# nekopanda/Amatsukaze

Hardware: AMD Instinct MI355X
Metric: frames/sec 1440x1080i logo+CM+KFM pass (higher is better)
Workload: dtype f32; 1 GPU; configs[1]: 10000x 1440x1080i 8-bit in HBM: AMTAnalyzeLogo, LogoFrame scan x3, CM/KFM metrics, CalcFade, AMTEraseLogo; analysis_mode=linear, library_default_mode=exact, calc_fade=device, erase=into a resident writable copy (MakeWritable's frame), frames_per_gpu=10000, logo=256x128@(1120,64), parallelism=single GPU

## Files before the change

### amatsukaze_amd/csrc/eval_engine.hip

```cpp
#include "build_knobs.h"
#include "engine.hpp"

#include <algorithm>
#include <cmath>
#include <cstdio>
#include <cstdlib>
#include <cstring>

int AmtGpuContext::prof_id(const char* name)
{
    for (size_t i = 0; i < prof_names.size(); ++i) if (prof_names[i] == name) return (int)i;
    prof_names.push_back(name);
    prof_ms.push_back(0.0);
    prof_calls.push_back(0);
    return (int)prof_names.size() - 1;
}
hipEvent_t AmtGpuContext::prof_event()
{
    if (!prof_pool.empty()) { hipEvent_t e = prof_pool.back(); prof_pool.pop_back(); return e; }
    hipEvent_t e;
    AMT_HIP(hipEventCreate(&e));
    return e;
}
int AmtGpuContext::prof_begin(const char* name)
// ... 89 lines not shown
                if ((slot_y(e) + 2 - ytop + 1) * lpb > kPlaneCapMax) break;
                minx = mnx; maxx = mxx;
                B.x0 = x0; B.bw = x1 - x0; B.lp = lpb;
                ++e;
            }
            if (e == s) throw std::runtime_error("logo too wide for the evaluation kernel");
            B.nslots = e - s;
            B.y0 = ytop;
            B.nrows = slot_y(e - 1) + 2 - ytop + 1;
            B.m0 = slot_m0(s);
            B.npix = slot_m0(e - 1) + (int)(slots[e - 1] >> 28) - B.m0;
            plane_cap_ = std::max(plane_cap_, B.nrows * B.lp);
            bands_.push_back(B);
            s = e;
        }

        std::vector<float2> scales((size_t)kNumBins * cpad, float2{0.0f, 0.0f});
        for (int m = 0; m < T.count; ++m)
            for (int c = 0; c < kNumBins; ++c)
                scales[(size_t)c * cpad + m] = float2{T.scales[((size_t)m * 32 + c) * 2], T.scales[((size_t)m * 32 + c) * 2 + 1]};
        const int spad = std::max(64, (ns + 63) / 64 * 64);
        std::vector<float2> kslot((size_t)25 * spad, float2{0.0f, 0.0f});
        std::vector<uint2> slot2(spad, uint2{0u, 0u});
        for (int bi = band0; bi < (int)bands_.size(); ++bi) {
            const EvalBand& B = bands_[bi];
            for (int sidx = B.s0; sidx < B.s0 + B.nslots; ++sidx) {
                const int m0 = slot_m0(sidx);
                const int n = (int)(slots[sidx] >> 28);
                const int x = (int)(T.pos[m0] & 0xFFFF), y = (int)(T.pos[m0] >> 16);
                slot2[sidx] = uint2{slots[sidx], (uint32_t)((y - 2 - B.y0) * B.lp + (x - 2 - B.x0))};
                const float* k0 = &T.kernels[(size_t)m0 * 25];
                const float* k1 = n > 1 ? &T.kernels[(size_t)(m0 + 1) * 25] : nullptr;
                for (int c = 0; c < 5; ++c)
                    for (int r = 0; r < 5; ++r) {
                        const float a0 = c < 4 ? k0[r * 5 + c + 1] : k0[r * 5];
                        const float a1 = k1 ? (c < 4 ? k1[r * 5 + c] : k1[r * 5 + 4]) : 0.0f;
                        kslot[(size_t)(c * 5 + r) * spad + sidx] = float2{a0, a1};
                    }
            }
        }
        d_a_[i].upload(S.planes.A(0), (size_t)w * h, ctx_->stream);
        d_b_[i].upload(S.planes.B(0), (size_t)w * h, ctx_->stream);
        d_scales_[i].upload(scales, ctx_->stream);
        d_kslot_[i].upload(kslot, ctx_->stream);
        d_slot2_[i].upload(slot2, ctx_->stream);

        EvalLogoDev& D = hl[i];
        D.a = d_a_[i].get(); D.b = d_b_[i].get(); D.scales = d_scales_[i].get();
        D.kslot = d_kslot_[i].get(); D.slot2 = d_slot2_[i].get(); D.nslots_pad = spad;
        D.band0 = band0; D.nbands = (int)bands_.size() - band0;
        D.w = w; D.h = h; D.count = T.count; D.count_pad = cpad;
        D.imgx = S.imgx; D.imgy = S.imgy; D.row0 = S.row0; D.row_step = S.row_step; D.deint = S.deint;
        D.blackScore = T.blackScore;
        D.out_off = S.out_off;
        D.lp = lp;
    }
#ifdef AMT_EXPERIMENT
    if (std::getenv("AMTGPU_VERBOSE")) {
        for (int i = 0; i < nl; ++i)
            fprintf(stderr, "[amtgpu] eval logo %d: %dx%d count=%d bands=%d lp=%d\n", i, hl[i].w, hl[i].h, hl[i].count, hl[i].nbands, hl[i].lp);
        for (const EvalBand& B : bands_)
            fprintf(stderr, "[amtgpu]   band logo=%d slots=%d npix=%d y0=%d nrows=%d x0=%d bw=%d lp=%d\n", B.logo, B.nslots, B.npix, B.y0, B.nrows, B.x0, B.bw, B.lp);
    }
#endif
    d_logos_.upload(hl, ctx_->stream);
    d_bands_.upload(bands_, ctx_->stream);
    d_fades_.upload(fades_, ctx_->stream);
}

double EvalEngine::mask_pixel_evals_per_frame() const
{
    double s = 0;
    for (const auto& sp : specs_) s += (double)sp.tables.count * fades_.size();
    return s;
}

void EvalEngine::run(const void* dY, int64_t frame_stride_bytes, int pitch, int bits, int nframes, float* dout,
                     const int* dframe_map)
{
    if (nframes <= 0 || specs_.empty()) return;
    ctx_->bind();
    const int es = bits <= 8 ? 1 : 2;
    if (frame_stride_bytes % es) throw std::runtime_error("frame stride not a multiple of the sample size");
    const int nl = (int)specs_.size();
    int G = exact_group_frames(nframes);
    const int nf_all = (int)fades_.size();
    if (pair_eligible() && pair_addressable(pitch * es)) {
        const size_t dot = prof_name_.find('.');
        const int sp = ctx_->prof_begin(("logo_eval_pair_kernel" + (dot == std::string::npos ? std::string() : prof_name_.substr(dot))).c_str());
        const int Gp = group_frames_ > 0 ? group_frames_ : (int)std::max(1LL, std::min((long long)kTileMaxFrames, (long long)nframes * nl / 2048));
        AMT_HIP(launch_logo_eval_pair(ctx_->stream, bits, d_logos_.get(), d_tls_.get(), nl, dY, dframe_map,
                                      frame_stride_bytes / es, pitch, nframes, Gp, dout, out_frame_stride_, take_abs_ ? 1 : 0));
        ctx_->prof_end(sp);
        return;
    }
    for (int f0 = 0; f0 < nf_all; f0 += kEvalMaxFades) {
        const int nf = std::min(kEvalMaxFades, nf_all - f0);
        G = std::max(1, std::min(G, kEvalThreads / nf));
        const int sp = ctx_->prof_begin(prof_name_.c_str());
        AMT_HIP(launch_logo_eval_fused(ctx_->stream, bits, d_logos_.get(), nl, d_bands_.get(), d_fades_.get(), nf, f0, dY, dframe_map,
                                       frame_stride_bytes / es, pitch, nframes, G, dout, out_frame_stride_, take_abs_ ? 1 : 0,
                                       plane_cap_));
        ctx_->prof_end(sp);
    }
}

int EvalEngine::exact_group_frames(int nframes) const
{
    const int nl = (int)specs_.size();
    return group_frames_ > 0 ? group_frames_ : (int)std::max(1LL, std::min(8LL, (long long)nframes * nl / 2048));
}

bool EvalEngine::pair_eligible()
{
    if (pair_state_ >= 0) return pair_state_ == 1;
    pair_state_ = 0;
#ifdef AMT_EXPERIMENT
    if (std::getenv("AMTGPU_NO_PAIR")) return false;
#endif
    if (fades_.size() != 2 || fades_[0] != 0.0f || fades_[1] != 1.0f || specs_.empty()) return false;
    for (const EvalLogoSpec& S : specs_) {
        const int w = S.planes.w, h = S.planes.h;
        if (w < 6 || (w & 1) || h < 5 || S.tables.count <= 0 || S.tables.count >= (1 << 20)) return false;
        if (!S.deint) return false;
        const float* a = S.planes.A(0);
        const float* b = S.planes.B(0);
        for (int p = 0; p < w * h; ++p)
            if (!(std::fabs(a[p]) + std::fabs(b[p]) < 8192.0f)) return false;
    }
    ensure_tiles();
    pair_state_ = 1;
    return true;
}

bool EvalEngine::pair_addressable(int pitch_bytes) const
{
    for (const EvalLogoSpec& S : specs_) {
        const long long last = (long long)(S.imgy + S.row0 + (long long)S.planes.h * S.row_step + 1) * pitch_bytes + (long long)(S.imgx + S.planes.w) * 2;
        if (last >= (1LL << 31) || pitch_bytes <= 0) return false;
    }
    return true;
}

void EvalEngine::ensure_tiles()
{
    if (tiles_ready_) return;
    ctx_->bind();
    const int nl = (int)specs_.size();
    std::vector<TileLogoDev> hl(nl);
    d_tkp_.resize(nl); d_tsc_.resize(nl); d_tpq_.resize(nl); d_tinfo_.resize(nl); d_tpos_.resize(nl); d_tlin_.resize(nl); d_tiles_.resize(nl); d_tbands_.resize(nl); d_tlist_.resize(nl);
    for (int i = 0; i < nl; ++i) {
        const EvalLogoSpec& S = specs_[i];
        const MaskTables& T = S.tables;
        const TilePlan P = build_tile_plan(T.pos, T.count, S.planes.w, S.planes.h);
        const size_t ns = (size_t)P.nslots();
        std::vector<float2> kp(13 * ns, float2{0.0f, 0.0f}), sc((size_t)kNumBins * ns, float2{0.0f, 0.0f}), pq(ns, float2{0.0f, 0.0f});
        std::vector<uint32_t> spos(ns, 0u);
        for (size_t s = 0; s < ns; ++s) {
            const int m = P.slot_pixel[s];
            if (m < 0) continue;
            fit_response(&T.resp[(size_t)m * 32], pq[s].x, pq[s].y);
            spos[s] = T.pos[m];
            const float* k = &T.kernels[(size_t)m * 25];
            float ksum = 0.0f;
            for (int t = 0; t < 25; ++t) ksum += k[t];
            for (int j = 0; j < 13; ++j) kp[(size_t)j * ns + s] = float2{k[2 * j], 2 * j + 1 < 25 ? k[2 * j + 1] : ksum};
            for (int c = 0; c < kNumBins; ++c)
                sc[(size_t)c * ns + s] = float2{T.scales[((size_t)m * 32 + c) * 2], T.scales[((size_t)m * 32 + c) * 2 + 1]};
        }
        d_tkp_[i].upload(kp, ctx_->stream);
        d_tsc_[i].upload(sc, ctx_->stream);
        d_tpq_[i].upload(pq, ctx_->stream);
        d_tpos_[i].upload(spos, ctx_->stream);
        const size_t npx = (size_t)S.planes.w * S.planes.h;
        const size_t o_pq = kp.size() * sizeof(float2), o_si = o_pq + pq.size() * sizeof(float2), o_a = o_si + P.sinfo.size() * sizeof(uint32_t),
                     o_b = o_a + npx * sizeof(float), total = o_b + npx * sizeof(float);
        if (total >= ((size_t)1 << 31)) throw std::runtime_error("logo too large");
        std::vector<char> blob(total);
        std::memcpy(blob.data(), kp.data(), o_pq);
        std::memcpy(blob.data() + o_pq, pq.data(), o_si - o_pq);
        std::memcpy(blob.data() + o_si, P.sinfo.data(), o_a - o_si);
        std::memcpy(blob.data() + o_a, S.planes.A(0), npx * sizeof(float));
        std::memcpy(blob.data() + o_b, S.planes.B(0), npx * sizeof(float));
        d_tlin_[i].upload(blob, ctx_->stream);
        d_tinfo_[i].upload(P.sinfo, ctx_->stream);
        d_tiles_[i].upload(P.tiles, ctx_->stream);
        d_tbands_[i].upload(P.bands, ctx_->stream);
        std::vector<int> tlist;
        for (size_t t = 0; t < P.tiles.size(); ++t) if (P.tiles[t].npix > 0) tlist.push_back((int)t);
        d_tlist_[i].upload(tlist, ctx_->stream);
        hl[i] = TileLogoDev{d_tkp_[i].get(), d_tsc_[i].get(), d_tpq_[i].get(), d_tinfo_[i].get(), d_tpos_[i].get(), d_tiles_[i].get(), d_tbands_[i].get(), d_tlist_[i].get(),
                            (int)P.bands.size(), (int)ns, (int)tlist.size(), T.floorResp};
        hl[i].lin = d_tlin_[i].get();
        hl[i].lin_pq = (unsigned)o_pq; hl[i].lin_sinfo = (unsigned)o_si; hl[i].lin_a = (unsigned)o_a; hl[i].lin_b = (unsigned)o_b;
    }
    d_tls_.upload(hl, ctx_->stream);
    tiles_ready_ = true;
}

void EvalEngine::ensure_linear()
{
    if (linear_ready_) return;
    const int nl = (int)specs_.size();
    lin_err_corr_.assign(nl, 0.0); lin_err_sum_.assign(nl, 0.0); lin_err_formula_.assign(nl, 0.0);
    lin_formula_ok_ = true;
    double vunit = 1.0;
    for (int i = 0; i < nl; ++i) {
        const EvalLogoSpec& S = specs_[i];
        const MaskTables& T = S.tables;
        const int w = S.planes.w, h = S.planes.h;
        const float* a = S.planes.A(0);
        const float* b = S.planes.B(0);
        for (int p = 0; p < w * h; ++p) {
            const double ab = (double)std::fabs(a[p]) + std::fabs(b[p]);
            if (!(ab < 1e30)) throw std::runtime_error("logo coefficients are not finite: the linear mode has no error bound for them");
            vunit = std::max(vunit, ab);
        }
        const double L = T.floorResp;
        if (!(L > 1e-20 && L < 1e30) || T.resp.size() != (size_t)T.count * 32) lin_formula_ok_ = false;
        double ecorr = 0, tsum = 0, eformula = 0;
        for (int m = 0; m < T.count; ++m) {
            double sk = 0;
            for (int t = 0; t < 25; ++t) sk += std::fabs(T.kernels[(size_t)m * 25 + t]);
            double smax = 0, s2max = 0, devmax = 0;
            float Pf = 0.0f, Qf = 0.0f;
            if (lin_formula_ok_) fit_response(&T.resp[(size_t)m * 32], Pf, Qf);
            if (!(std::fabs(Pf) < 1e30f && std::fabs(Qf) < 1e30f)) lin_formula_ok_ = false;
            for (int c = 0; c < kNumBins; ++c) {
                const double sc = std::fabs(T.scales[((size_t)m * 32 + c) * 2]), s2 = std::fabs(T.scales[((size_t)m * 32 + c) * 2 + 1]);
                smax = std::max(smax, sc * s2);
                s2max = std::max(s2max, s2);
                if (!lin_formula_ok_) continue;
                const double rk = formula_response(Pf, Qf, c), dk = std::max(rk, L);
                const auto tref = [&](double x) { return std::min(1.0, x * sc) * s2; };
                const auto tker = [&](double x) { return std::min(x, rk) / dk; };
                double dev = std::fabs((sc > 0 ? s2 : 0.0) - rk / dk);
                dev = std::max(dev, std::fabs(tref(rk) - tker(rk)));
                if (sc > 0) dev = std::max(dev, std::fabs(tref(1.0 / sc) - tker(1.0 / sc)));
                devmax = std::max(devmax, dev);
                smax = std::max(smax, 1.0 / dk);
                s2max = std::max(s2max, rk / dk);
            }
            eformula += devmax;
            ecorr += smax * sk * (58.0 + 24.0);
            tsum += s2max;
        }
        const double black = std::max(1e-30, (double)std::fabs(T.blackScore));
        lin_err_corr_[i] = ecorr / black;
        lin_err_sum_[i] = ((double)T.count + 52.0) * tsum / black + 8.0;
        lin_err_formula_[i] = eformula / black;
    }
    bool unit_fades = true;
    for (float f : fades_) unit_fades = unit_fades && f >= 0.0f && f <= 1.0f;
    vmax_unit_ = (float)(vunit * (unit_fades ? 1.0 : 2.0));
    linear_ready_ = true;
}

bool EvalEngine::tiles_usable(int pitch_bytes) const
{
    for (const EvalLogoSpec& S : specs_) {
        const int w = S.planes.w, h = S.planes.h;
        if (w < 6 || (w & 1) || h < 5 || S.tables.count <= 0 || S.tables.count >= 900000) return false;
    }
    return pair_addressable(pitch_bytes);
}

float EvalEngine::linear_error_bound(int logo, int bits) const
{
    const_cast<EvalEngine*>(this)->ensure_linear();
    const double u = 1.0 / 16777216.0, maxv = (double)((1 << bits) - 1);
    return (float)(1.25 * (u * (lin_err_corr_[logo] * vmax_unit_ * maxv + lin_err_sum_[logo]) + lin_err_formula_[logo]));
}

void EvalEngine::run_linear(const void* dY, int64_t frame_stride_bytes, int pitch, int bits, int nframes, float* dout, const int* dframe_map,
                            uint8_t* dforce)
{
    if (nframes <= 0 || specs_.empty()) return;
    const int es = bits <= 8 ? 1 : 2;
    if ((int)fades_.size() != 11 || fades_.front() != 0.0f || fades_.back() != 1.0f || !tiles_usable(pitch * es)) { run(dY, frame_stride_bytes, pitch, bits, nframes, dout, dframe_map); return; }
    ensure_linear();
    if (!lin_formula_ok_) { run(dY, frame_stride_bytes, pitch, bits, nframes, dout, dframe_map); return; }
    ensure_tiles();
    ctx_->bind();
    if (frame_stride_bytes % es) throw std::runtime_error("frame stride not a multiple of the sample size");
    const int nl = (int)specs_.size();
    const double vwin = (double)vmax_unit_ * (double)((1 << bits) - 1);
    const float bin_eps = (float)(22.0 / 16777216.0 * vwin * 1.0001);
    int qlog2 = 24;
    while (qlog2 > 4 && std::ldexp(vwin, qlog2) >= 1073741824.0) --qlog2;
    if (!(std::ldexp(vwin, qlog2) < 1073741824.0)) { run(dY, frame_stride_bytes, pitch, bits, nframes, dout, dframe_map); return; }
    const int qcap = std::max(16, std::min(640, lin_queue_));
    const int g_fit = (int)((160 * 1024 / 4 - 16 * 1024 - 4 * 8 * qcap - 16) / (4 * 768));
    if (g_fit < 1) { run(dY, frame_stride_bytes, pitch, bits, nframes, dout, dframe_map); return; }
    const int gmax = std::min(g_fit, bits > 8 ? kLinMaxFrames16 : kLinMaxFrames);
    const long long wgs_min = bits > 8 ? AMT_LIN_WGS_MIN16 : 2048;
    const int G = std::min(gmax, group_frames_ > 0 ? group_frames_ : (int)std::max(1LL, std::min(16LL, (long long)nframes * nl / wgs_min)));
    const size_t dot = prof_name_.find('.');
    const int sp = ctx_->prof_begin(("logo_eval_linear_kernel" + (dot == std::string::npos ? std::string() : prof_name_.substr(dot))).c_str());
    AMT_HIP(launch_logo_eval_linear(ctx_->stream, bits, d_logos_.get(), d_tls_.get(), nl, d_fades_.get(), 11, 0, dY, dframe_map,
                                    frame_stride_bytes / es, pitch, nframes, G, dout, out_frame_stride_, take_abs_ ? 1 : 0, bin_eps, qlog2,
                                    qcap, dforce));
    ctx_->prof_end(sp);
}

#ifndef AMT_LISTED_FADE_CHUNK
#define AMT_LISTED_FADE_CHUNK 1
#endif
// ... 23 lines not shown
```

### amatsukaze_amd/csrc/eval_pair_kernels.hip

```cpp
#include "build_knobs.h"
#include <hip/hip_runtime.h>
#include <cstdint>
#include <algorithm>

#include "engine.hpp"
#include "eval_tiles.hpp"
#include "exact_math.h"
#include "eval_tile_stage.h"
#include "eval_ordered_sum.h"

namespace amt {

using namespace lin;
using namespace tile;

constexpr int kPairThreads = (kTileWaves + 1) * 64;
constexpr int kPairRowPitch = kTileBandPix + kEvalScorePad;

__device__ __forceinline__ f2 window_corr_exact(const f2 (&Kp)[13], const f2 (&W)[25], f2 M)
{
    f2 p[5];
#pragma unroll
    for (int i = 0; i < 5; ++i) {
        f2 t[5];
#pragma unroll
        for (int r = 0; r < 5; ++r) {
            const int e = r * 5 + i;
            const f2 kk = (e & 1) ? bc_hi(Kp[e >> 1]) : bc_lo(Kp[e >> 1]);
            t[r] = kk * (W[e] - M);
        }
        p[i] = ((t[0] + t[1]) + (t[2] + t[3])) + t[4];
    }
    return ((p[0] + p[4]) + p[2]) + (p[1] + p[3]);
}

__device__ __forceinline__ unsigned score_bin_bounded(float mean) { return (unsigned)((int)__builtin_amdgcn_fmed3f(mean, 0.0f, 255.0f) >> 3); }

struct PairLaunch {
    const EvalLogoDev* logos;
    const TileLogoDev* tls;
    const void* Y;
    const int* frame_map;
    long long frame_stride;
    int pitch;
    float maxv;
    int nframes, G, ngroups, nlogos;
    float* out;
    int out_frame_stride, take_abs;
};

#ifdef AMT_PAIR_OCC
#define AMT_PAIR_OCC_ATTR __attribute__((amdgpu_waves_per_eu(AMT_PAIR_OCC, AMT_PAIR_OCC)))
#else
#define AMT_PAIR_OCC_ATTR
#endif
template <typename pix_t>
__global__ __launch_bounds__(kPairThreads) AMT_PAIR_OCC_ATTR
void logo_eval_pair_kernel(const PairLaunch A)
{
    extern __shared__ float lds[];
    f2* const planes = reinterpret_cast<f2*>(lds);
    float* const rows = lds + kTileWaves * kTileCap * 2;

#ifdef AMT_PAIR_TIMING
    long long tacc[8] = {0, 0, 0, 0, 0, 0, 0, 0};
    long long tprev = clock64();
#define AMT_PTICK(k) do { const long long t_ = clock64(); tacc[k] += t_ - tprev; tprev = t_; } while (0)
#define AMT_PDUMP() do { if (lane == 0 && logo == 0 && grp == A.ngroups / 2) { \
        long long* tb = reinterpret_cast<long long*>(A.out + (long long)A.nframes * A.out_frame_stride);    \
        for (int k = 0; k < 8; ++k) tb[wave * 8 + k] = tacc[k]; \
        tb[16 * 8 + wave] = __builtin_amdgcn_s_getreg((4 << 0) | (0 << 6) | (31 << 11));    } } while (0)
#else
#define AMT_PTICK(k) do { } while (0)
#define AMT_PDUMP() do { } while (0)
#endif
    const int G = A.G;
    const WgMap wm = wg_map_shared_rows((int)blockIdx.x, A.nlogos, A.ngroups);
    if (wm.grp >= A.ngroups) return;
    const int logo = wm.logo, grp = wm.grp;
    const int F0 = grp * G;
    const int gcount = min(G, A.nframes - F0);
    const int tid = threadIdx.x, lane = tid & 63;
    const int wave = __builtin_amdgcn_readfirstlane(tid >> 6);
    const EvalLogoDev* const Lp = A.logos + logo;
    const TileLogoDev* const Xp = A.tls + logo;
    const int nbands = Xp->nbands;
    constexpr int ES = (int)sizeof(pix_t);

    if (wave == kTileWaves) {
        __builtin_amdgcn_s_setprio(3);
        float acc = 0.0f;
        typedef const __attribute__((address_space(4))) TileBandDesc* const_band_ptr;
        const const_band_ptr bd = (const_band_ptr)Xp->bands;
        for (int b = 0; b < nbands; ++b) {
            asm volatile("s_waitcnt lgkmcnt(0)\n\ts_barrier" ::: "memory");
            AMT_PTICK(5);
            const int npix = bd[b].npix;
#ifndef AMT_PAIR_NO_SUM
            if (lane < 2 * gcount) acc = ordered_row_sum(rows + ((b & 1) * 2 * G + lane) * kPairRowPitch, npix, acc);
#endif
#ifdef AMT_PAIR_TIMING
            asm volatile("" : "+v"(acc));
#endif
            AMT_PTICK(0);
        }
        if (lane < 2 * gcount) {
            float r = acc / Lp->blackScore;
            if (A.take_abs) r = fabsf(r);
            A.out[(long long)(F0 + (lane >> 1)) * A.out_frame_stride + Lp->out_off + (lane & 1)] = r;
        }
        AMT_PDUMP();
        return;
    }

    const gptr_t gSc = (gptr_t)Xp->sc;
    const unsigned nslots8 = (unsigned)Xp->nslots * 8u;
    const const_tile_ptr tiles = (const_tile_ptr)(Xp->tiles + wave);
    f2* const myplane = planes + wave * kTileCap;
    const unsigned plane_base = lds_address(myplane);
    TileStager<pix_t> st;
    st.init(Lp, A.pitch, A.maxv, myplane);
    TilePixel px;

    TileDesc T;
    fetch_tile(T, tiles);
    st.setup_units(T, lane);
    st.request(frame_rsrc<pix_t>(A.Y, A.frame_map, A.frame_stride, F0));
    asm volatile("" ::: "memory");
    px.load(Xp, (unsigned)wave * 64u + (unsigned)lane, T, plane_base);

    f2 pR = {0.0f, 0.0f}, psc0 = pR, psc1 = pR;
    int prow = 0;
    bool pact = false;
    auto flush_terms = [&]() {
        if (pact) {
            float* const pdst = rows + prow * kPairRowPitch + px.ridx;
            pdst[0] = score_term(pR.x, psc0.x, psc0.y);
            pdst[kPairRowPitch] = score_term(pR.y, psc1.x, psc1.y);
        }
    };

    int b = 0, g = 0;
    const int niter = nbands * gcount;
    for (int it = 0; it < niter; ++it) {
        const bool band_end = g + 1 == gcount;
        AMT_PTICK(6);
#ifdef AMT_PAIR_TIMING
        asm volatile("s_waitcnt vmcnt(2)" ::: "memory");
        AMT_PTICK(7);
#endif
#ifndef AMT_PAIR_NO_CONVERT
        st.convert();
#endif
        AMT_PTICK(0);
        if (band_end && b + 1 < nbands) {
            fetch_tile(T, tiles + (b + 1) * kTileWaves);
            st.setup_units(T, lane);
        }
#if defined(AMT_PAIR_RAW_SAMEFRAME)
        st.request(frame_rsrc<pix_t>(A.Y, A.frame_map, A.frame_stride, 0));
#elif !defined(AMT_PAIR_NO_RAW)
        st.request(frame_rsrc<pix_t>(A.Y, A.frame_map, A.frame_stride, F0 + (band_end ? 0 : g + 1)));
#endif
        AMT_PTICK(1);
#pragma unroll
        for (int j = 0; j < 13; ++j) asm volatile("" : "+v"(px.Kp[j]));
        f2 W[25];
        unsigned wrow[5];
        px.rows(wrow);
#ifdef AMT_PAIR_NO_EVAL
        const f2 M = px.Kp[1] + f2{100.0f, 120.0f}, R = px.Kp[0];
        (void)W;
#else
        const f2 M = window_load_means(wrow, W);
        const f2 R = window_corr_exact(px.Kp, W, M);
#endif
#ifdef AMT_PAIR_TIMING
        { f2 Rt = R; asm volatile("" : "+v"(Rt)); }
#endif
        AMT_PTICK(2);
#ifndef AMT_PAIR_NO_FLUSH
        flush_terms();
#endif
#ifdef AMT_PAIR_NO_GATHER
        psc0 = f2{1e-3f, 1.0f} + M; psc1 = f2{1e-3f, 1.0f} - M;
#else
        psc0 = gld<f2>(gSc, __umul24(score_bin_bounded(M.x), nslots8) + px.slot8);
        psc1 = gld<f2>(gSc, __umul24(score_bin_bounded(M.y), nslots8) + px.slot8);
#endif
        pR = R; pact = px.act;
        AMT_PTICK(3);
        prow = (b & 1) * 2 * G + g * 2;
        if (band_end) {
            flush_terms();
            pact = false;
            ++b; g = 0;
            if (b < nbands) px.load(Xp, (unsigned)(b * kTileWaves + wave) * 64u + (unsigned)lane, T, plane_base);
            AMT_PTICK(4);
            asm volatile("s_waitcnt lgkmcnt(0)\n\ts_barrier" ::: "memory");
            AMT_PTICK(5);
        } else {
            ++g;
        }
    }
    AMT_PDUMP();
}

hipError_t launch_logo_eval_pair(hipStream_t st, int bits, const EvalLogoDev* dlogos, const TileLogoDev* dtls, int nlogos,
                                 const void* dY, const int* dframe_map, long long frame_stride_elems, int pitch,
                                 int nframes, int G, float* dout, int out_frame_stride, int take_abs)
{
    if (nframes <= 0 || nlogos <= 0) return hipSuccess;
    PairLaunch A;
    A.logos = dlogos; A.tls = dtls; A.Y = dY; A.frame_map = dframe_map; A.frame_stride = frame_stride_elems; A.pitch = pitch;
    A.maxv = (float)((1 << bits) - 1);
    A.nframes = nframes; A.G = G; A.ngroups = (nframes + G - 1) / G; A.nlogos = nlogos;
    A.out = dout; A.out_frame_stride = out_frame_stride; A.take_abs = take_abs;
    const size_t lds = ((size_t)kTileWaves * kTileCap * 2 + (size_t)2 * 2 * G * kPairRowPitch) * sizeof(float);
    if (G < 1 || 2 * G > 64 || lds > 160 * 1024) return hipErrorInvalidValue;
    dim3 grid((unsigned)wg_grid_shared_rows(A.ngroups, nlogos));
    if (bits <= 8) hipLaunchKernelGGL(logo_eval_pair_kernel<uint8_t>, grid, dim3(kPairThreads), lds, st, A);
    else hipLaunchKernelGGL(logo_eval_pair_kernel<uint16_t>, grid, dim3(kPairThreads), lds, st, A);
    return hipGetLastError();
}

}
```

### amatsukaze_amd/csrc/eval_tile_stage.h

```cpp
#pragma once
#include <hip/hip_runtime.h>
#include <cstdint>

#include "engine.hpp"
#include "eval_tiles.hpp"
#include "exact_math.h"
#include "eval_lds_stage.h"

namespace amt {

namespace tile {

using namespace lin;

__device__ __forceinline__ void window_reads(const unsigned (&wrow)[5], f2 (&W)[25])
{
#pragma unroll
    for (int r = 0; r < 5; ++r)
        asm volatile("ds_read_b64 %0, %5\n\tds_read_b64 %1, %5 offset:8\n\tds_read_b64 %2, %5 offset:16\n\t"
                     "ds_read_b64 %3, %5 offset:24\n\tds_read_b64 %4, %5 offset:32"
                     : "=&v"(W[5 * r]), "=&v"(W[5 * r + 1]), "=&v"(W[5 * r + 2]), "=&v"(W[5 * r + 3]), "=&v"(W[5 * r + 4])
                     : "v"(wrow[r]) : "memory");
}
template <int OUTSTANDING, int ROW0, int NROWS>
// ... 72 lines not shown
    f2 W[25];
    window_reads(wrow, W);
    f2 acc0 = {0.0f, 0.0f}, acc1 = acc0, c[5];
    auto mac = [&](int e) {
        if (e & 1) acc1 = pk_fma_tap(1, e == 1, Kp[e >> 1], W[e], acc1);
        else acc0 = pk_fma_tap(0, e == 0, Kp[e >> 1], W[e], acc0);
    };
    window_rows_ready<15, 0, 2>(W);
#pragma unroll
    for (int i = 0; i < 5; ++i) c[i] = W[i] + W[5 + i];
#pragma unroll
    for (int e = 0; e < 10; ++e) mac(e);
    window_rows_ready<5, 2, 2>(W);
#pragma unroll
    for (int i = 0; i < 5; ++i) c[i] = c[i] + (W[10 + i] + W[15 + i]);
#pragma unroll
    for (int e = 10; e < 20; ++e) mac(e);
    window_rows_ready<0, 4, 1>(W);
#pragma unroll
    for (int i = 0; i < 5; ++i) c[i] = c[i] + W[20 + i];
#pragma unroll
    for (int e = 20; e < 25; ++e) mac(e);
    M = div25_pk(((c[0] + c[4]) + c[2]) + (c[1] + c[3]));
    const f2 sum = acc0 + acc1;
    asm("v_pk_fma_f32 %0, %1, %2, %3 op_sel:[1,0,0] neg_lo:[1,0,0] neg_hi:[1,0,0]" : "=v"(R) : "v"(Kp[12]), "v"(M), "v"(sum));
}
template <bool ONE_TRIP>
__device__ __forceinline__ void window_eval_streamed(const unsigned (&wrow)[5], const f2 (&Kp)[13], f2& M, f2& R)
{
    if (ONE_TRIP) { window_eval_one_trip(wrow, Kp, M, R); return; }
    f2 ra[10];
    window_rows_issue2(wrow[0], wrow[1], ra);
    f2 acc0 = {0.0f, 0.0f}, acc1 = acc0, c[5];
    auto mac = [&](int e, f2 wv) {
        if (e & 1) acc1 = pk_fma_tap(1, e == 1, Kp[e >> 1], wv, acc1);
        else acc0 = pk_fma_tap(0, e == 0, Kp[e >> 1], wv, acc0);
    };
    rows_ready2<0>(ra);
#pragma unroll
    for (int i = 0; i < 5; ++i) c[i] = ra[i] + ra[5 + i];
#pragma unroll
    for (int e = 0; e < 10; ++e) mac(e, ra[e]);
    window_rows_issue2(wrow[2], wrow[3], ra);
    rows_ready2<0>(ra);
#pragma unroll
    for (int i = 0; i < 5; ++i) c[i] = c[i] + (ra[i] + ra[5 + i]);
#pragma unroll
    for (int e = 0; e < 10; ++e) mac(10 + e, ra[e]);
    f2 r4[5];
    window_row_issue1(wrow[4], r4);
    row_ready1<0>(r4);
#pragma unroll
    for (int i = 0; i < 5; ++i) c[i] = c[i] + r4[i];
#pragma unroll
    for (int e = 0; e < 5; ++e) mac(20 + e, r4[e]);
    M = div25_pk(((c[0] + c[4]) + c[2]) + (c[1] + c[3]));
    {
        const f2 sum = acc0 + acc1;
        asm("v_pk_fma_f32 %0, %1, %2, %3 op_sel:[1,0,0] neg_lo:[1,0,0] neg_hi:[1,0,0]" : "=v"(R) : "v"(Kp[12]), "v"(M), "v"(sum));
    }
}

template <typename pix_t> struct Quad;
template <> struct Quad<uint8_t> {
    unsigned v;
    __device__ __forceinline__ void load(__amdgpu_buffer_rsrc_t r, int voff) { v = __builtin_amdgcn_raw_buffer_load_b32(r, voff, 0, 0); }
    static __device__ __forceinline__ void blend(const Quad& r0, const Quad& r1, const Quad& r2, unsigned bias, float (&s)[4])
    {
        const unsigned e0 = __builtin_amdgcn_perm(r0.v, r0.v, 0x0C020C00u), o0 = __builtin_amdgcn_perm(r0.v, r0.v, 0x0C030C01u);
        const unsigned e1 = __builtin_amdgcn_perm(r1.v, r1.v, 0x0C020C00u), o1 = __builtin_amdgcn_perm(r1.v, r1.v, 0x0C030C01u);
        const unsigned e2 = __builtin_amdgcn_perm(r2.v, r2.v, 0x0C020C00u), o2 = __builtin_amdgcn_perm(r2.v, r2.v, 0x0C030C01u);
        unsigned te, to;
        asm("v_lshl_add_u32 %0, %1, 1, %2" : "=v"(te) : "v"(e1), "v"(e0));
        asm("v_lshl_add_u32 %0, %1, 1, %2" : "=v"(to) : "v"(o1), "v"(o0));
        const unsigned se = te + e2 + bias;
        const unsigned so = to + o2 + bias;
        s[0] = __builtin_amdgcn_ldexpf((float)(se & 0xFFFFu), -2);
        s[1] = __builtin_amdgcn_ldexpf((float)(so & 0xFFFFu), -2);
        s[2] = __builtin_amdgcn_ldexpf((float)(se >> 16), -2);
        s[3] = __builtin_amdgcn_ldexpf((float)(so >> 16), -2);
    }
    static constexpr unsigned kBias = 0x00020002u;
    static __device__ __forceinline__ void copy(const Quad& r1, float (&s)[4])
    {
        s[0] = (float)(r1.v & 0xFFu); s[1] = (float)((r1.v >> 8) & 0xFFu); s[2] = (float)((r1.v >> 16) & 0xFFu); s[3] = (float)(r1.v >> 24);
    }
};
template <> struct Quad<uint16_t> {
    u2 v;
    __device__ __forceinline__ void load(__amdgpu_buffer_rsrc_t r, int voff) { v = __builtin_amdgcn_raw_buffer_load_b64(r, voff, 0, 0); }
    static __device__ __forceinline__ void blend(const Quad& r0, const Quad& r1, const Quad& r2, unsigned bias, float (&s)[4])
    {
#pragma unroll
        for (int k = 0; k < 4; ++k) {
            const unsigned a = (r0.v[k >> 1] >> (16 * (k & 1))) & 0xFFFFu, b = (r1.v[k >> 1] >> (16 * (k & 1))) & 0xFFFFu,
                           c = (r2.v[k >> 1] >> (16 * (k & 1))) & 0xFFFFu;
            s[k] = __builtin_amdgcn_ldexpf((float)(((b << 1) + a) + (c + bias)), -2);
        }
    }
    static constexpr unsigned kBias = 2u;
    static __device__ __forceinline__ void copy(const Quad& r1, float (&s)[4])
    {
#pragma unroll
        for (int k = 0; k < 4; ++k) s[k] = (float)((r1.v[k >> 1] >> (16 * (k & 1))) & 0xFFFFu);
    }
};

typedef const __attribute__((address_space(4))) TileDesc* const_tile_ptr;
typedef const __attribute__((address_space(4))) int* const_int_ptr;
__device__ __forceinline__ void fetch_tile(TileDesc& D, const_tile_ptr t)
{
    D.x0 = t->x0; D.y0 = t->y0; D.nrows = t->nrows; D.ncol4 = t->ncol4; D.tp = t->tp; D.npix = t->npix; D.rcp = t->rcp;
}

template <typename pix_t, bool AB_LDS = false, bool SLIM = false, bool BLEND = true> struct TileStager {
    static constexpr int ES = (int)sizeof(pix_t);
    int w, h, deint, srow0, srow_step, scol0, pitchB;
    float maxv;
    gptr_t gA, gB;
    f2* plane;
    f2* abplane;
    bool second_pass;
    int ulds[kTileUnits];
    int ug[kTileUnits][3];
    unsigned ubias[kTileUnits];
    f4 ua[kTileUnits], ubmv[kTileUnits];
    Quad<pix_t> raw[kTileUnits][3];

    __device__ __forceinline__ void init(const EvalLogoDev* Lp, int pitch, float maxv_, f2* plane_, f2* abplane_ = nullptr)
    {
        abplane = abplane_;
        w = Lp->w; h = Lp->h; deint = Lp->deint;
        srow0 = Lp->imgy + Lp->row0; srow_step = Lp->row_step; scol0 = Lp->imgx;
        gA = (gptr_t)Lp->a; gB = (gptr_t)Lp->b;
        pitchB = pitch * ES; maxv = maxv_; plane = plane_;
        second_pass = false;
    }
    __device__ __forceinline__ void setup_units(const TileDesc& T, int lane)
    {
        second_pass = T.nrows * T.ncol4 > 64;
#pragma unroll
        for (int k = 0; k < kTileUnits; ++k) {
            const TileUnit U = tile_unit(T, lane + 64 * k, w);
            const bool blend = BLEND && deint && U.y > 0 && U.y < h - 1;
            ulds[k] = SLIM ? (U.lds | (blend ? (int)0x80000000 : 0)) : U.lds;
            if (!SLIM) ubias[k] = blend ? Quad<pix_t>::kBias : 0u;
            ug[k][1] = (srow0 + U.y * srow_step) * pitchB + (scol0 + U.xs) * ES;
            if (!SLIM) {
                ug[k][0] = blend ? ug[k][1] - pitchB : ug[k][1];
                ug[k][2] = blend ? ug[k][1] + pitchB : ug[k][1];
            }
            typedef f4 __attribute__((aligned(8))) f4a8;
            const f4 av = gld<f4a8>(gA, (unsigned)(U.y * w + U.xs) * 4u);
            const f4 bmv = gld<f4a8>(gB, (unsigned)(U.y * w + U.xs) * 4u) * maxv;
            if (AB_LDS) {
                f4* d = reinterpret_cast<f4*>(abplane + U.lds);
                d[0] = f4{av[0], bmv[0], av[1], bmv[1]};
                d[1] = f4{av[2], bmv[2], av[3], bmv[3]};
            } else {
                ua[k] = av; ubmv[k] = bmv;
            }
        }
    }
    __device__ __forceinline__ void request(const __amdgpu_buffer_rsrc_t frame)
    {
#pragma unroll
        for (int k = 0; k < kTileUnits; ++k) {
            if (!BLEND) {
                raw[k][1].load(frame, ug[k][1]);
            } else if (SLIM) {
                const int d = (ulds[k] >> 31) & pitchB;
                raw[k][0].load(frame, ug[k][1] - d);
                raw[k][1].load(frame, ug[k][1]);
                raw[k][2].load(frame, ug[k][1] + d);
            } else {
#pragma unroll
                for (int j = 0; j < 3; ++j) raw[k][j].load(frame, ug[k][j]);
            }
        }
    }
    __device__ __forceinline__ void convert_unit(int k)
    {
        float sv[4];
        const unsigned bias = SLIM ? ((unsigned)(ulds[k] >> 31) & Quad<pix_t>::kBias) : ubias[k];
        const int lds = SLIM ? (ulds[k] & 0x7FFFFFFF) : ulds[k];
        if (BLEND) Quad<pix_t>::blend(raw[k][0], raw[k][1], raw[k][2], bias, sv);
        else Quad<pix_t>::copy(raw[k][1], sv);
        f2* dst = plane + lds;
        if (AB_LDS) {
            const f4* c = reinterpret_cast<const f4*>(abplane + lds);
            const f4 c0 = c[0], c1 = c[1];
            reinterpret_cast<f4*>(dst)[0] = f4{sv[0], c0[0] * sv[0] + c0[1], sv[1], c0[2] * sv[1] + c0[3]};
            reinterpret_cast<f4*>(dst)[1] = f4{sv[2], c1[0] * sv[2] + c1[1], sv[3], c1[2] * sv[3] + c1[3]};
        } else {
            reinterpret_cast<f4*>(dst)[0] = f4{sv[0], ua[k][0] * sv[0] + ubmv[k][0], sv[1], ua[k][1] * sv[1] + ubmv[k][1]};
            reinterpret_cast<f4*>(dst)[1] = f4{sv[2], ua[k][2] * sv[2] + ubmv[k][2], sv[3], ua[k][3] * sv[3] + ubmv[k][3]};
        }
    }
    __device__ __forceinline__ void convert()
    {
        convert_unit(0);
        if (second_pass) {
#pragma unroll
            for (int k = 1; k < kTileUnits; ++k) convert_unit(k);
        }
    }
};

template <typename pix_t>
__device__ __forceinline__ __amdgpu_buffer_rsrc_t frame_rsrc(const void* Y, const int* frame_map, long long frame_stride, int frame)
{
    const int srcFrame = frame_map ? ((const_int_ptr)frame_map)[frame] : frame;
    const pix_t* src = reinterpret_cast<const pix_t*>(Y) + (long long)srcFrame * frame_stride;
    return __builtin_amdgcn_make_buffer_rsrc(const_cast<pix_t*>(src), 0, 0x7FFFFFFF, 0x00020000);
}

struct TilePixel {
    f2 Kp[13];
    unsigned w0;
    unsigned tp8;
    int ridx;
    bool act;
    unsigned slot8;
    unsigned slotbase8;
    __device__ __forceinline__ void load(const TileLogoDev* Xp, unsigned slot, const TileDesc& T, unsigned plane_base)
    {
        const gptr_t gK = (gptr_t)Xp->kp, gInfo = (gptr_t)Xp->sinfo;
        const unsigned nslots8 = (unsigned)Xp->nslots * 8u;
        const unsigned si = gld<unsigned>(gInfo, slot * 4u);
        w0 = plane_base + (si & 0xFFFu) * 8u;
        tp8 = (unsigned)T.tp * 8u;
        ridx = (int)((si >> 12) & 0xFFFu);
        act = (si >> 31) != 0;
        slot8 = slot * 8u;
        slotbase8 = __builtin_amdgcn_readfirstlane(slot8);
#pragma unroll
        for (int j = 0; j < 13; ++j) Kp[j] = gld<f2>(gK, (unsigned)j * nslots8 + slot8);
    }
    __device__ __forceinline__ void rows(unsigned (&wrow)[5]) const
    {
#pragma unroll
        for (int r = 0; r < 5; ++r) wrow[r] = w0 + (unsigned)r * tp8;
    }
};

__device__ __forceinline__ unsigned lds_address(const void* p)
{
    return (unsigned)(unsigned long long)(__attribute__((address_space(3))) const char*)p;
}

}

}
```

### amatsukaze_amd/csrc/eval_tiles.hpp

```cpp
#pragma once

#include <algorithm>
#include <cstdint>
#include <stdexcept>
#include <vector>

namespace amt {

#ifndef AMT_TILE_WAVES
#define AMT_TILE_WAVES 11
#endif
constexpr int kTileWaves = AMT_TILE_WAVES;
#ifndef AMT_TILE_G
#define AMT_TILE_G 8
#endif
constexpr int kTileMaxFrames = AMT_TILE_G;
constexpr int kTileLanes = 64;
constexpr int kTileBandPix = kTileWaves * kTileLanes;
constexpr int kTileCap = 512;
constexpr int kTileUnits = kTileCap / 4 / kTileLanes;

struct TileDesc {
    int x0, y0;
    int nrows, ncol4;
    int tp;
    int npix;
    int rcp;
    int pad;
};
struct TileBandDesc {
    int m0, npix;
};
#if defined(__HIPCC__)
#define AMT_TILE_HD __host__ __device__ inline __attribute__((always_inline))
#else
#define AMT_TILE_HD inline
#endif
struct TileUnit { int y, xs, lds; };
AMT_TILE_HD TileUnit tile_unit(const TileDesc& T, int u, int w)
{
    const int last = T.nrows * T.ncol4 - 1;
    u = u < last ? u : (last < 0 ? 0 : last);
    const int row = (u * T.rcp) >> 16;
    const int c4 = u - row * T.ncol4;
    const int x = T.x0 + 4 * c4;
    const int xs = x < w - 4 ? x : w - 4;
    return TileUnit{T.y0 + row, xs, row * T.tp + (xs - T.x0)};
}

constexpr int kXcds = 8;
struct WgMap { int logo, grp; };
AMT_TILE_HD WgMap wg_map_shared_rows(int bid, int nlogos, int ngroups)
{
#ifdef AMT_WG_PLAIN_MAP
    if (bid >= nlogos * ngroups) return WgMap{0, ngroups};
    return WgMap{bid / ngroups, bid % ngroups};
#endif
    (void)ngroups;
    const int x = bid & (kXcds - 1), r = bid >> 3;
    const int blk = r / nlogos;
    return WgMap{r - blk * nlogos, blk * kXcds + x};
}
inline long long wg_grid_shared_rows(long long ngroups, int nlogos) { return (ngroups + kXcds - 1) / kXcds * kXcds * nlogos; }

inline uint32_t tile_slot_info(int woff, int ridx, bool valid) { return (uint32_t)woff | ((uint32_t)ridx << 12) | (valid ? 0x80000000u : 0u); }

struct TilePlan {
    std::vector<TileBandDesc> bands;
    std::vector<TileDesc> tiles;
    std::vector<uint32_t> sinfo;
    std::vector<int> slot_pixel;
    int nslots() const { return (int)sinfo.size(); }
};

namespace tiles_detail {

struct Px { int x, y, m; };

inline int split_lanes(const std::vector<Px>& g, int x0, int y0, int tp, std::vector<uint8_t>* half)
{
    const int n = (int)g.size();
    int k[32] = {0};
    std::vector<int> bank(n);
    for (int i = 0; i < n; ++i) { bank[i] = ((g[i].y - 2 - y0) * tp + (g[i].x - 2 - x0)) & 31; ++k[bank[i]]; }
    for (int total = 2;; ++total)
        for (int ca = (total + 1) / 2; ca < total; ++ca) {
            const int cb = total - ca;
            int lo = 0, hi = 0;
            bool ok = true;
            for (int b = 0; b < 32; ++b) { ok = ok && k[b] <= total; lo += std::max(0, k[b] - cb); hi += std::min(k[b], ca); }
            const int smin = std::max(lo, n - 32), smax = std::min(hi, 32);
            if (!ok || smin > smax) continue;
            if (half) {
                int a[32], sum = 0;
                for (int b = 0; b < 32; ++b) { a[b] = std::max(0, k[b] - cb); sum += a[b]; }
                const int want = std::min(std::max((n + 1) / 2, smin), smax);
                for (bool moved = true; sum < want && moved;) {
                    moved = false;
                    for (int b = 0; b < 32 && sum < want; ++b)
                        if (a[b] < std::min(k[b], ca)) { ++a[b]; ++sum; moved = true; }
                }
                half->assign(n, 1);
                for (int i = 0; i < n; ++i)
                    if (a[bank[i]] > 0) { (*half)[i] = 0; --a[bank[i]]; }
            }
            return total;
        }
}

struct Geometry { int x0, y0, nrows, ncol4; };
inline Geometry bbox(const std::vector<Px>& g, size_t a, size_t b)
{
    int xmin = 1 << 30, xmax = -1, ymin = 1 << 30, ymax = -1;
    for (size_t i = a; i < b; ++i) {
        xmin = std::min(xmin, g[i].x); xmax = std::max(xmax, g[i].x);
        ymin = std::min(ymin, g[i].y); ymax = std::max(ymax, g[i].y);
    }
    Geometry G;
    G.x0 = (xmin - 2) & ~1;
    G.y0 = ymin - 2;
    G.nrows = ymax + 2 - G.y0 + 1;
    G.ncol4 = (xmax + 2 - G.x0 + 1 + 3) / 4;
    return G;
}
inline bool fits(const Geometry& G) { return G.nrows * G.ncol4 * 4 <= kTileCap && G.nrows * G.ncol4 <= kTileLanes * kTileUnits; }

}

inline TilePlan build_tile_plan(const std::vector<uint32_t>& pos, int count, int w, int h)
{
    using namespace tiles_detail;
    (void)h;
    if (w < 5) throw std::runtime_error("logo too narrow for the tile kernel");
    TilePlan P;
    for (int m = 0; m < count;) {
        int n = std::min(kTileBandPix, count - m);
        std::vector<std::vector<Px>> groups;
        for (;;) {
            std::vector<Px> px(n);
            for (int i = 0; i < n; ++i) px[i] = Px{(int)(pos[m + i] & 0xFFFFu), (int)(pos[m + i] >> 16), m + i};
            std::stable_sort(px.begin(), px.end(), [](const Px& a, const Px& b) { return a.x < b.x; });
            groups.clear();
            for (size_t a = 0; a < px.size();) {
                size_t b = a + 1;
                while (b < px.size() && b - a < (size_t)kTileLanes && fits(bbox(px, a, b + 1))) ++b;
                groups.emplace_back(px.begin() + a, px.begin() + b);
                a = b;
            }
            if ((int)groups.size() <= kTileWaves) break;
            n = std::max(1, n - std::max(1, n / 8));
        }
        {
            std::vector<size_t> order(groups.size());
            for (size_t i = 0; i < order.size(); ++i) order[i] = i;
            auto cost = [&](size_t i) { const Geometry G = bbox(groups[i], 0, groups[i].size()); return 131 + 31 * (G.nrows * G.ncol4 > kTileLanes ? 2 : 1); };
            std::stable_sort(order.begin(), order.end(), [&](size_t a, size_t b) { return cost(a) > cost(b); });
            int load[4] = {0, 0, 0, 0}, used[4] = {0, 0, 0, 0}, cap[4] = {0, 0, 0, 0};
            for (int w = 0; w < kTileWaves; ++w) ++cap[w % 4];
            std::vector<std::vector<Px>> placed(kTileWaves);
            for (size_t i : order) {
                int best = -1;
                for (int k = 0; k < 4; ++k)
                    if (used[k] < cap[k] && (best < 0 || load[k] < load[best])) best = k;
                placed[best + 4 * used[best]] = groups[i];
                load[best] += cost(i); ++used[best];
            }
            groups.swap(placed);
        }
        const int band = (int)P.bands.size();
        P.bands.push_back(TileBandDesc{m, n});
        P.tiles.resize((size_t)(band + 1) * kTileWaves, TileDesc{0, 0, 0, 1, 4, 0, 65536, 0});
        P.sinfo.resize((size_t)(band + 1) * kTileBandPix, tile_slot_info(0, 0, false));
        P.slot_pixel.resize((size_t)(band + 1) * kTileBandPix, -1);
        for (size_t gi = 0; gi < groups.size(); ++gi) {
            const std::vector<Px>& g = groups[gi];
            if (g.empty()) continue;
            const Geometry G = bbox(g, 0, g.size());
            int best_tp = G.ncol4 * 4, best_cyc = 1 << 30;
            for (int tp = G.ncol4 * 4; tp * G.nrows <= kTileCap && tp < G.ncol4 * 4 + 32; tp += 2) {
                const int c = split_lanes(g, G.x0, G.y0, tp, nullptr);
                if (c < best_cyc) { best_cyc = c; best_tp = tp; }
            }
            std::vector<uint8_t> half;
            split_lanes(g, G.x0, G.y0, best_tp, &half);
            TileDesc& T = P.tiles[(size_t)band * kTileWaves + gi];
            T.x0 = G.x0; T.y0 = G.y0; T.nrows = G.nrows; T.ncol4 = G.ncol4; T.tp = best_tp; T.npix = (int)g.size();
            T.rcp = (65536 + G.ncol4 - 1) / G.ncol4;
            for (int u = 0; u < kTileLanes * kTileUnits; ++u)
                if (((u * T.rcp) >> 16) != u / G.ncol4) throw std::runtime_error("tile plan: unit row magic");
            int next[2] = {0, kTileLanes / 2}, filler[2] = {-1, -1};
            for (size_t i = 0; i < g.size(); ++i) {
                const int l = next[half[i]]++;
                const size_t slot = ((size_t)band * kTileWaves + gi) * kTileLanes + l;
                const int woff = (g[i].y - 2 - G.y0) * best_tp + (g[i].x - 2 - G.x0);
                if (l >= kTileLanes / 2 * (half[i] + 1)) throw std::runtime_error("tile plan: more than 32 pixels in half a wave");
                if (woff < 0 || woff + 4 * best_tp + 4 > G.nrows * best_tp - 1 || G.nrows * best_tp > kTileCap) throw std::runtime_error("tile plan: window outside its tile");
                P.sinfo[slot] = tile_slot_info(woff, g[i].m - m, true);
                P.slot_pixel[slot] = g[i].m;
                if (filler[half[i]] < 0) filler[half[i]] = woff;
            }
            for (int hf = 0; hf < 2; ++hf) {
                const int woff = filler[hf] >= 0 ? filler[hf] : filler[1 - hf];
                for (int l = next[hf]; l < kTileLanes / 2 * (hf + 1); ++l)
                    P.sinfo[((size_t)band * kTileWaves + gi) * kTileLanes + l] = tile_slot_info(woff, 0, false);
            }
        }
        m += n;
    }
    return P;
}

}
```

Before: 1.251 million frames/sec.

## Choose band cuts by modeled cost and defer coefficient scaling past loads

The tile planner is refactored so band cutting can use a coarse or a finer step-by-4 cut, with a merge of a small tail band. When two fades are present it builds both plans and keeps the one with lower modeled per-SIMD load. The kernel also hoists the kp/sinfo pointers through the constant address space and postpones the maxv multiply on register-held B coefficients until after the pixel load is issued, so the load does not wait on that multiply. The extra plan build adds host setup time, and the cost model may not match real kernel time.

```diff
diff --git a/amatsukaze_amd/csrc/eval_engine.hip b/amatsukaze_amd/csrc/eval_engine.hip
--- a/amatsukaze_amd/csrc/eval_engine.hip
+++ b/amatsukaze_amd/csrc/eval_engine.hip
@@ -265,7 +265,7 @@
     for (int i = 0; i < nl; ++i) {
         const EvalLogoSpec& S = specs_[i];
         const MaskTables& T = S.tables;
-        const TilePlan P = build_tile_plan(T.pos, T.count, S.planes.w, S.planes.h);
+        const TilePlan P = build_tile_plan(T.pos, T.count, S.planes.w, S.planes.h, fades_.size() == 2 ? kTileCutBest : kTileCutCoarse);
         const size_t ns = (size_t)P.nslots();
         std::vector<float2> kp(13 * ns, float2{0.0f, 0.0f}), sc((size_t)kNumBins * ns, float2{0.0f, 0.0f}), pq(ns, float2{0.0f, 0.0f});
         std::vector<uint32_t> spos(ns, 0u);
diff --git a/amatsukaze_amd/csrc/eval_pair_kernels.hip b/amatsukaze_amd/csrc/eval_pair_kernels.hip
--- a/amatsukaze_amd/csrc/eval_pair_kernels.hip
+++ b/amatsukaze_amd/csrc/eval_pair_kernels.hip
@@ -113,7 +113,8 @@
         return;
     }
 
-    const gptr_t gSc = (gptr_t)Xp->sc;
+    typedef const __attribute__((address_space(4))) TileLogoDev* tlogo_ptr;
+    const gptr_t gSc = (gptr_t)Xp->sc, gK = (gptr_t)((tlogo_ptr)Xp)->kp, gInfo = (gptr_t)((tlogo_ptr)Xp)->sinfo;
     const unsigned nslots8 = (unsigned)Xp->nslots * 8u;
     const const_tile_ptr tiles = (const_tile_ptr)(Xp->tiles + wave);
     f2* const myplane = planes + wave * kTileCap;
@@ -127,7 +128,8 @@
     st.setup_units(T, lane);
     st.request(frame_rsrc<pix_t>(A.Y, A.frame_map, A.frame_stride, F0));
     asm volatile("" ::: "memory");
-    px.load(Xp, (unsigned)wave * 64u + (unsigned)lane, T, plane_base);
+    px.load(gK, gInfo, nslots8, (unsigned)wave * 64u + (unsigned)lane, T, plane_base);
+    st.coefs_landed();
 
     f2 pR = {0.0f, 0.0f}, psc0 = pR, psc1 = pR;
     int prow = 0;
@@ -195,7 +197,10 @@
             flush_terms();
             pact = false;
             ++b; g = 0;
-            if (b < nbands) px.load(Xp, (unsigned)(b * kTileWaves + wave) * 64u + (unsigned)lane, T, plane_base);
+            if (b < nbands) {
+                st.coefs_landed();
+                px.load(gK, gInfo, nslots8, (unsigned)(b * kTileWaves + wave) * 64u + (unsigned)lane, T, plane_base);
+            }
             AMT_PTICK(4);
             asm volatile("s_waitcnt lgkmcnt(0)\n\ts_barrier" ::: "memory");
             AMT_PTICK(5);
diff --git a/amatsukaze_amd/csrc/eval_tile_stage.h b/amatsukaze_amd/csrc/eval_tile_stage.h
--- a/amatsukaze_amd/csrc/eval_tile_stage.h
+++ b/amatsukaze_amd/csrc/eval_tile_stage.h
@@ -248,14 +248,22 @@
             }
             typedef f4 __attribute__((aligned(8))) f4a8;
             const f4 av = gld<f4a8>(gA, (unsigned)(U.y * w + U.xs) * 4u);
-            const f4 bmv = gld<f4a8>(gB, (unsigned)(U.y * w + U.xs) * 4u) * maxv;
+            f4 bmv = gld<f4a8>(gB, (unsigned)(U.y * w + U.xs) * 4u);
             if (AB_LDS) {
+                bmv = bmv * maxv;
                 f4* d = reinterpret_cast<f4*>(abplane + U.lds);
                 d[0] = f4{av[0], bmv[0], av[1], bmv[1]};
                 d[1] = f4{av[2], bmv[2], av[3], bmv[3]};
             } else {
                 ua[k] = av; ubmv[k] = bmv;
             }
+        }
+    }
+    __device__ __forceinline__ void coefs_landed()
+    {
+        if (!AB_LDS) {
+#pragma unroll
+            for (int k = 0; k < kTileUnits; ++k) ubmv[k] = ubmv[k] * maxv;
         }
     }
     __device__ __forceinline__ void request(const __amdgpu_buffer_rsrc_t frame)
@@ -319,10 +327,8 @@
     bool act;
     unsigned slot8;
     unsigned slotbase8;
-    __device__ __forceinline__ void load(const TileLogoDev* Xp, unsigned slot, const TileDesc& T, unsigned plane_base)
-    {
-        const gptr_t gK = (gptr_t)Xp->kp, gInfo = (gptr_t)Xp->sinfo;
-        const unsigned nslots8 = (unsigned)Xp->nslots * 8u;
+    __device__ __forceinline__ void load(gptr_t gK, gptr_t gInfo, unsigned nslots8, unsigned slot, const TileDesc& T, unsigned plane_base)
+    {
         const unsigned si = gld<unsigned>(gInfo, slot * 4u);
         w0 = plane_base + (si & 0xFFFu) * 8u;
         tp8 = (unsigned)T.tp * 8u;
diff --git a/amatsukaze_amd/csrc/eval_tiles.hpp b/amatsukaze_amd/csrc/eval_tiles.hpp
--- a/amatsukaze_amd/csrc/eval_tiles.hpp
+++ b/amatsukaze_amd/csrc/eval_tiles.hpp
@@ -70,8 +70,10 @@
     std::vector<TileDesc> tiles;
     std::vector<uint32_t> sinfo;
     std::vector<int> slot_pixel;
+    long long model_cost = 0;
     int nslots() const { return (int)sinfo.size(); }
 };
+enum TileCut { kTileCutCoarse, kTileCutFine, kTileCutBest };
 
 namespace tiles_detail {
 
@@ -127,29 +129,54 @@
 
 }
 
-inline TilePlan build_tile_plan(const std::vector<uint32_t>& pos, int count, int w, int h)
+namespace tiles_detail {
+
+inline std::vector<std::vector<Px>> deal_band(const std::vector<uint32_t>& pos, int m, int n)
+{
+    std::vector<Px> px(n);
+    for (int i = 0; i < n; ++i) px[i] = Px{(int)(pos[m + i] & 0xFFFFu), (int)(pos[m + i] >> 16), m + i};
+    std::stable_sort(px.begin(), px.end(), [](const Px& a, const Px& b) { return a.x < b.x; });
+    std::vector<std::vector<Px>> groups;
+    for (size_t a = 0; a < px.size();) {
+        size_t b = a + 1;
+        while (b < px.size() && b - a < (size_t)kTileLanes && fits(bbox(px, a, b + 1))) ++b;
+        groups.emplace_back(px.begin() + a, px.begin() + b);
+        a = b;
+    }
+    return groups;
+}
+inline std::vector<int> cut_bands(const std::vector<uint32_t>& pos, int count, bool fine)
+{
+    std::vector<int> cuts;
+    for (int m = 0; m < count;) {
+        int n = std::min(kTileBandPix, count - m);
+        while ((int)deal_band(pos, m, n).size() > kTileWaves)
+            n = fine ? std::max(1, n - 4) : std::max(1, n - std::max(1, n / 8));
+        cuts.push_back(n);
+        m += n;
+    }
+    if (fine && cuts.size() >= 2 && cuts.back() < kTileLanes) {
+        const int n = cuts[cuts.size() - 2] + cuts.back();
+        if (n <= kTileBandPix && (int)deal_band(pos, count - n, n).size() <= kTileWaves) { cuts.pop_back(); cuts.back() = n; }
+    }
+    return cuts;
+}
+
+}
+
+inline TilePlan build_tile_plan(const std::vector<uint32_t>& pos, int count, int w, int h, TileCut cut = kTileCutCoarse)
 {
     using namespace tiles_detail;
     (void)h;
     if (w < 5) throw std::runtime_error("logo too narrow for the tile kernel");
+    if (cut == kTileCutBest) {
+        TilePlan coarse = build_tile_plan(pos, count, w, h, kTileCutCoarse), fine = build_tile_plan(pos, count, w, h, kTileCutFine);
+        return fine.model_cost < coarse.model_cost ? fine : coarse;
+    }
     TilePlan P;
-    for (int m = 0; m < count;) {
-        int n = std::min(kTileBandPix, count - m);
-        std::vector<std::vector<Px>> groups;
-        for (;;) {
-            std::vector<Px> px(n);
-            for (int i = 0; i < n; ++i) px[i] = Px{(int)(pos[m + i] & 0xFFFFu), (int)(pos[m + i] >> 16), m + i};
-            std::stable_sort(px.begin(), px.end(), [](const Px& a, const Px& b) { return a.x < b.x; });
-            groups.clear();
-            for (size_t a = 0; a < px.size();) {
-                size_t b = a + 1;
-                while (b < px.size() && b - a < (size_t)kTileLanes && fits(bbox(px, a, b + 1))) ++b;
-                groups.emplace_back(px.begin() + a, px.begin() + b);
-                a = b;
-            }
-            if ((int)groups.size() <= kTileWaves) break;
-            n = std::max(1, n - std::max(1, n / 8));
-        }
+    int m = 0;
+    for (const int n : cut_bands(pos, count, cut == kTileCutFine)) {
+        std::vector<std::vector<Px>> groups = deal_band(pos, m, n);
         {
             std::vector<size_t> order(groups.size());
             for (size_t i = 0; i < order.size(); ++i) order[i] = i;
@@ -165,6 +192,7 @@
                 placed[best + 4 * used[best]] = groups[i];
                 load[best] += cost(i); ++used[best];
             }
+            P.model_cost += *std::max_element(load, load + 4);
             groups.swap(placed);
         }
         const int band = (int)P.bands.size();
```

After: 1.270 million frames/sec (median of 6 runs). 1.6% higher.
